# abacus-gene/paml

Hardware: AMD Instinct MI355X
Metric: site-patterns/sec per lnL eval (codeml M0, 61 states) (higher is better)
Workload: dtype f64; 1 GPU; codeml M0 61-state, 16 taxa x 1000000 synthetic codon patterns sharded over the GPUs (BASELINE configs[3]); classes=1, kernel=mfma64_jit, parallelism=pattern-shard x1, RCCL all-reduce inside the engine, patterns_rank0=1000000

## Files before the change

### include/paml_amd.h

```cpp
#ifndef PAML_AMD_H
#define PAML_AMD_H

#ifdef __cplusplus
extern "C" {
#endif

typedef struct paml_amd_engine paml_amd_engine;

enum {
   PAML_AMD_OK = 0,
   PAML_AMD_EINVAL = -1,
   PAML_AMD_ENOMEM = -2,
   PAML_AMD_EHIP = -3,
   PAML_AMD_EUNSUPPORTED = -4,
   PAML_AMD_ENOCONV = -5
};

enum {
   PAML_AMD_KEEP_PARTIALS = 1,
   PAML_AMD_JIT = 2,
   PAML_AMD_SHARD = 4
};

enum { PAML_AMD_EIGEN_UVROOT = 0, PAML_AMD_EIGEN_CIJK = 1, PAML_AMD_EIGEN_K80 = 2, PAML_AMD_EIGEN_JC69LIKE = 3, PAML_AMD_EIGEN_QMAT = 4 };
// ... 68 lines not shown
                        const double *qfactor, const double *freqK, const double *rate, double *lnL, double *lnf);

int paml_amd_eval_branch(paml_amd_engine *e, int node_b, int n_t, const double *t, const double *branch,
                         const double *gene_rate, double *lnL, double *dlnL, double *ddlnL);
int paml_amd_branch_counters(const paml_amd_engine *e, long *n_calls, long *n_nodes_recomputed);
long paml_amd_branch_coef_hits(const paml_amd_engine *e);
long paml_amd_branch_refill_kernels(const paml_amd_engine *e);
double paml_amd_branch_kernel_ms(paml_amd_engine *e);
int paml_amd_get_branch_partials(paml_amd_engine *e, double *out, long cap, long *rows, int *cols);

int paml_amd_node_posterior(paml_amd_engine *e, int node, const double *branch, const double *gene_rate, double *post);

int paml_amd_get_pmat(paml_amd_engine *e, int gene, int iclass, int node, double *P);
int paml_amd_get_partials(paml_amd_engine *e, int node, int iclass, double *conP);
int paml_amd_get_scale(paml_amd_engine *e, int node, int iclass, double *scale);
int paml_amd_get_partial_sums(paml_amd_engine *e, double *out, int cap);

int paml_amd_profile(paml_amd_engine *e, int enable);
int paml_amd_profile_read(paml_amd_engine *e, double *ms_pmat, double *ms_prune, double *ms_reduce, long *n_evals);

int paml_amd_counters(const paml_amd_engine *e, long *n_eval, long *n_pmat);

int paml_amd_cherry_tables(const paml_amd_engine *e, long *n_tabulated, long *bytes);
int paml_amd_subtree_tables(const paml_amd_engine *e, long *n_tabulated, int *nodes, long *u, int cap, long *bytes, long *blocks_left, long *n_computed);
int paml_amd_subtree_order(const paml_amd_engine *e, int *in_use, long *n_computed, double *host_seconds);
int paml_amd_gather_walk(const paml_amd_engine *e, int *in_use, long *n_tiles, long *n_rows, int *R, long *n_computed, double *host_seconds);

int paml_amd_debug_program(int n_tips, int n_nodes, int root, const int *sons_ptr, const int *sons,
                           const unsigned char *scale_node, int keep_partials, const unsigned char *clean,
                           int *ops_out, int cap, int *max_stack);

int paml_amd_debug_branch_plan(int n_tips, int n_nodes, int root, const int *sons_ptr, const int *sons, const unsigned char *scale_node,
                               int n_calls, const int *node_b, const double *branch, int *ends_out, int *up_out, unsigned char *clean_out,
                               int *ops_out, int cap);

int paml_amd_debug_code_order(int n_states, int n_codes, const int *n_chara, const unsigned char *chara_map, const unsigned char *z,
                              long nz, int *order_out);

int paml_amd_debug_jit(int n_tips, int n_nodes, int root, const int *sons_ptr, const int *sons,
                       const unsigned char *scale_node, char *text_out, int cap, int compile);

int paml_amd_debug_jit_tables(int n_tips, int n_nodes, int root, const int *sons_ptr, const int *sons, const unsigned char *scale_node,
                              int max_tabs, char *text_out, int cap, int *stream_out, int stream_cap, int *n_stream, int *tabs_out,
                              int tabs_cap);

int paml_amd_debug_subtree_classes(int n_tips, int n_nodes, int root, const int *sons_ptr, const int *sons, const unsigned char *z, long n_patt,
                                   int n_codes, unsigned int *u_out, unsigned int *cls_out);
// ... 141 lines not shown
```

### paml_amd/csrc/engine_core.hip

```cpp
#include "engine_state.h"
#include "eigen_kernels.h"

namespace paml_amd {
int launch_eigen_qrev(paml_amd_engine *e, EigenQrevArgs a, int n_sets)
{
   if (!e->eigen_attr_set) {
      for (const void *fn : {(const void *)eigen_qrev_kernel<0>, (const void *)eigen_qrev_kernel<20>, (const void *)eigen_qrev_kernel<60>, (const void *)eigen_qrev_kernel<62>})
         HIPCHK(hipFuncSetAttribute(fn, hipFuncAttributeMaxDynamicSharedMemorySize, (int)EIG_LDS_BYTES));
      e->eigen_attr_set = true;
   }
   static const int sweep_limit = getenv("PAML_AMD_EIGEN_SWEEP_LIMIT") ? std::max(1, atoi(getenv("PAML_AMD_EIGEN_SWEEP_LIMIT"))) : 40;
   a.max_sweeps = sweep_limit;
   const int N_even = (a.n + 1) & ~1;
   if (N_even == 62) hipLaunchKernelGGL(eigen_qrev_kernel<62>, dim3(n_sets), dim3(EIG_NT), EIG_LDS_BYTES, e->stream, a);
   else if (N_even == 60) hipLaunchKernelGGL(eigen_qrev_kernel<60>, dim3(n_sets), dim3(EIG_NT), EIG_LDS_BYTES, e->stream, a);
   else if (N_even == 20) hipLaunchKernelGGL(eigen_qrev_kernel<20>, dim3(n_sets), dim3(EIG_NT), EIG_LDS_BYTES, e->stream, a);
   else hipLaunchKernelGGL(eigen_qrev_kernel<0>, dim3(n_sets), dim3(EIG_NT), EIG_LDS_BYTES, e->stream, a);
   HIPCHK(hipGetLastError());
   return 0;
}
}

extern "C" {

// ... 680 lines not shown
   for (size_t i = 0; i + 5 < e->ev_used.size(); i += 6)
      for (int k = 0; k < 3; k++) {
         float ms = 0;
         if (hipEventElapsedTime(&ms, e->ev_used[i + 2 * k], e->ev_used[i + 2 * k + 1]) == hipSuccess) acc[k] += ms;
      }
   for (DevEvent &ev : e->ev_used) e->ev_pool.push_back(std::move(ev));
   e->ev_used.clear();
   if (ms_pmat) *ms_pmat = acc[0];
   if (ms_prune) *ms_prune = acc[1];
   if (ms_reduce) *ms_reduce = acc[2];
   if (n_evals) *n_evals = e->prof_evals;
   e->prof_evals = 0;
   return 0;
}

int paml_amd_cherry_tables(const paml_amd_engine *e, long *n_tabulated, long *bytes)
{
   if (!e) return PAML_AMD_EINVAL;
   if (n_tabulated) *n_tabulated = e->last_ctab_n;
   if (bytes) *bytes = e->last_ctab_bytes;
   return 0;
}

int paml_amd_subtree_tables(const paml_amd_engine *e, long *n_tabulated, int *nodes, long *u, int cap, long *bytes, long *blocks_left, long *n_computed)
{
   if (!e) return PAML_AMD_EINVAL;
   if (n_tabulated) *n_tabulated = e->last_stab_n;
   for (long i = 0; i < e->last_stab_n && i < cap && i < (long)e->sub.sel.size(); i++) {
      if (nodes) nodes[i] = e->sub.sel[i];
      if (u) u[i] = (long)e->sub.u[e->sub.sel[i]];
   }
   if (bytes) *bytes = e->last_stab_bytes;
   if (blocks_left) *blocks_left = e->last_stab_blocks;
   if (n_computed) *n_computed = e->sub.n_computed;
   return 0;
}

int paml_amd_subtree_order(const paml_amd_engine *e, int *in_use, long *n_computed, double *host_seconds)
{
   if (!e) return PAML_AMD_EINVAL;
   if (in_use) *in_use = (e->last_stab_n && e->sub.ordered) ? 1 : 0;
   if (n_computed) *n_computed = e->sub.n_order_computed;
   if (host_seconds) *host_seconds = e->sub.order_host_s;
   return 0;
}

int paml_amd_gather_walk(const paml_amd_engine *e, int *in_use, long *n_tiles, long *n_rows, int *R, long *n_computed, double *host_seconds)
{
   if (!e) return PAML_AMD_EINVAL;
// ... 19 lines not shown
```

### paml_amd/csrc/engine_eval.hip

```cpp
#include "engine_state.h"
#include "kernels_pmat.h"
#include "kernels_prune.h"
#include "kernels_reduce.h"

namespace paml_amd {

int build_tiles(paml_amd_engine *e)
{
   std::vector<int2> tiles;
   for (int g = 0; g < e->n_genes; g++)
      for (int h = e->gene_off[g]; h < e->gene_off[g + 1]; h += e->tile_patt) tiles.push_back(make_int2(g, h));
   e->n_tiles = (int)tiles.size();
   HIPCHK(upload(e->d_tiles, tiles.data(), tiles.size(), e->stream));
   const int tf = e->kk == KK_MFMA64 ? GATHER_WAVES * 16 : 256;
   std::vector<int2> tfull;
   for (int g = 0; g < e->n_genes; g++)
      for (int h = e->gene_off[g]; h < e->gene_off[g + 1]; h += tf) tfull.push_back(make_int2(g, h));
   e->n_tiles_full = (int)tfull.size();
   HIPCHK(upload(e->d_tiles_full, tfull.data(), tfull.size(), e->stream));
   if (e->kk == KK_MFMA64) {
      std::vector<int> g0(tiles.size());
      size_t k = 0;
      int base = 0;
      for (int g = 0; g < e->n_genes; g++) {
// ... 177 lines not shown
};

int begin_eval(paml_amd_engine *e, Eval &c)
{
   if (!(e->have_tips && e->have_tree && e->have_pi && e->have_classes))
      return fail(e, PAML_AMD_EINVAL, "eval before set_tips/set_tree/set_pi/set_classes");
   if (e->eigen.empty()) return fail(e, PAML_AMD_EINVAL, "eval before any set_eigen_*");
   c.keep = (e->flags & PAML_AMD_KEEP_PARTIALS) != 0;
   if (c.clean && (!c.keep || !e->partials_valid))
      return fail(e, PAML_AMD_EINVAL, "eval_dirty needs PAML_AMD_KEEP_PARTIALS and a previous full evaluation");
   c.B = c.bs ? c.bs->B : 1; c.Km = e->K; c.K = c.Km * c.B; c.G = e->n_genes; c.psets = c.G * c.K;
   if (c.B > 1 && (c.keep || c.clean)) return fail(e, PAML_AMD_EUNSUPPORTED, "eval_batch: not with PAML_AMD_KEEP_PARTIALS");
   c.new_prog = !e->prog_valid || c.clean;
   if (c.new_prog) {
      e->prog = build_program(e->tree, c.keep, c.clean);
      e->prog_valid = (c.clean == nullptr);
      if (int rc = check_stack_depth(e, e->prog)) { e->prog_valid = false; return rc; }
   }
   return 0;
}

int setup_streams(paml_amd_engine *e, Eval &c)
{
   c.want_pipe = c.want_pipe && (e->kk == KK_MFMA64 || (e->kk == KK_VALU20 && e->want_m20)) && (long)e->n_patt * e->K >= 100000;
   c.pipe = c.want_pipe && e->pipe_ok && !c.bs && !c.clean && !c.keep && !c.new_prog && !e->eigen_dirty;
   c.dual = c.pipe && e->dual_ok && !e->profiling;
   c.lane = c.dual ? e->red_slot : 0;
   if (c.dual && c.lane && !e->sb[c.lane - 1]) HIPCHK(create_engine_stream(&e->sb[c.lane - 1]));
   if (c.dual)
      if (int rc = ensure_side_stream(e)) return rc;
   c.ms = c.lane ? e->sb[c.lane - 1] : e->stream;
   if (c.want_pipe && !e->s2) {
      for (DevEvent &ev : e->ev_setread) HIPCHK(ev.ensure(hipEventDisableTiming));
      for (int i = 0; i < paml_amd_engine::NPSET - 1; i++) e->spare[i].id = i + 1;
      HIPCHK(create_engine_stream(&e->s2));
      HIPCHK(e->ev_entry[0].ensure(hipEventDisableTiming));
      HIPCHK(e->ev_entry[1].ensure(hipEventDisableTiming));
      HIPCHK(e->ev_pmat.ensure(hipEventDisableTiming));
   }
   c.ps = e->stream;
   if (c.pipe) {
      c.ps = e->s2;
      if (e->have_prev_entry && !(c.dual && e->dual_run)) HIPCHK(hipStreamWaitEvent(e->s2, e->ev_entry[e->entry_sel ^ 1], 0));
      const int nid = e->spare[e->spare_head].id;
      if (c.dual && e->setread_rec[nid]) HIPCHK(hipStreamWaitEvent(e->s2, e->ev_setread[nid], 0));
   }
   c.skip_entry = c.dual && e->dual_run;
   e->dual_run = c.dual;
   return 0;
}

int stage_inputs(paml_amd_engine *e, Eval &c, InlineVec &iv)
{
   const int B = c.B, Km = c.Km, G = c.G, nn = e->tree.n_nodes;
   const BatchSpec *const bs = c.bs;
   std::vector<EigenDev> tab;
// ... 377 lines not shown
         e->fused_threads = 256 * pl.CW;
      }
      if (!jit_ok) {
         int r = obtain_kernel(e, e->jit_slot, &e->jit, true, "v" + std::to_string(n) + ":" + jit_program_key(e->prog, e->n_tips),
                               [&]() { return jit_generate_valu(e->prog, n); }, JIT_WAIT_CALLER, "valu", &jit_ok);
         if (r) return r;
      }
   }
   if (e->want_m20 && !c.clean && jit_m20_supported(e->prog, e->n_tips, G)) {
      int r = obtain_kernel(e, e->jit_slot, &e->jit, true, std::string("m20c") + std::to_string(e->n_codes) + (G > 1 ? "g:" : ":") + jit_program_key(e->prog, e->n_tips),
                            [&]() { return jit_generate_m20(e->prog, e->n_tips, e->n_codes, G > 1 ? 2 : 1); }, JIT_WAIT_CALLER, "m20", &jit_ok);
      if (r) return r;
      second = jit_ok;
   }
   *out = PruneKernel(3 * e->kk + (second ? 2 : (jit_ok ? 1 : 0)));
   return 0;
}

int ensure_buffers(paml_amd_engine *e, Eval &c)
{
   if (c.pipe) {
      paml_amd_engine::PSet &sp = e->spare[e->spare_head];
      std::swap(e->d_rowmajor, sp.rowmajor); std::swap(e->d_pint, sp.pint); std::swap(e->d_ptip, sp.ptip); std::swap(e->d_pcol, sp.pcol);
      std::swap(e->d_ctab, sp.ctab);
      std::swap(e->d_stab, sp.stab);
      std::swap(e->pset, sp.id);
      e->spare_head = (e->spare_head + 1) % (paml_amd_engine::NPSET - 1);
   }
   if (int rc = ensure_pmat_buffers(e, c.psets, e->kk == KK_VALU20 && e->want_m20, e->kk == KK_MFMA64)) return rc;
   if (e->kernel != PK_MFMA64_JIT) e->n_ctab = e->n_stab = 0;
   e->last_stab_n = e->n_stab;
   e->last_stab_bytes = e->n_stab ? (long)((size_t)c.K * e->sub.rows * CHERRY_ROW_BYTES) : 0;
   e->last_stab_blocks = e->n_stab ? (long)(e->sub.sp.prog.stream.size() / 2) : -1;
   if (e->n_stab) HIPCHK(e->d_stab.ensure((size_t)e->last_stab_bytes / sizeof(double)));
   e->last_ctab_n = e->n_ctab;
   e->last_ctab_bytes = (long)((size_t)c.K * e->n_ctab * cherry_table_bytes(e->n_codes));
   if (e->n_ctab) HIPCHK(e->d_ctab.ensure((size_t)e->last_ctab_bytes / sizeof(double)));
   HIPCHK(e->d_fhK.ensure((size_t)c.K * e->n_patt));
   c.n_blocks = e->n_tiles * c.K;
   if (c.keep) {
      const int n_int = e->tree.n_nodes - e->n_tips;
      size_t words = e->kk == KK_MFMA64 ? (size_t)c.K * n_int * e->part_groups() * 1024 + (size_t)std::max(e->mfma_waves, 8) * 1024
                                        : (size_t)c.K * n_int * e->n_patt * e->n;
      HIPCHK(e->d_partials.ensure(words));
      HIPCHK(e->d_scalef.ensure((size_t)c.K * std::max(1, e->tree.n_scale) * e->n_patt));
   }
   return stack_overflow(e, e->prog, c.n_blocks, e->mfma_waves, &c.overflow);
}

int run_pmat(paml_amd_engine *e, Eval &c, const InlineVec &iv)
{
   const int B = c.B, Km = c.Km, G = c.G, nn = e->tree.n_nodes;
   const BatchSpec *const bs = c.bs;
   PmatArgs pa = pmat_args(e, e->tree.root, e->d_label.p, e->kk == KK_MFMA64 ? 1 : (e->kernel == PK_MFMA4X20_JIT ? 2 : 0),
                           e->kk == KK_MFMA64 ? e->d_pcol.p : nullptr);
   if (c.pipe) { pa.branch = e->d2_branch.p; pa.gene_rate = e->d2_gene_rate.p; }
   pa.B = B; pa.branch_bs = nn; pa.gene_rate_bs = G;
   if (bs && bs->eigen_of) { pa.eigen_of = e->d_b_eigen_of.p; pa.eigen_of_bs = (long)G * Km * e->n_labels; }
   if (bs && bs->qfactor) { pa.qfactor = e->d_b_qfactor.p; pa.qfactor_bs = (long)Km * e->n_labels; }
   pa.npb = 1;
// ... 4 lines not shown
   e->pmat_B = B;
   if (pmat_mfma && !bs && c.use_inline && !e->rate_per_gene && !e->eigen.empty()) {
      if (!e->pres_valid) {
         std::vector<PmatRes> res((size_t)c.psets * nn);
         for (int g = 0; g < G; g++)
            for (int ir = 0; ir < Km; ir++)
               for (int v = 0; v < nn; v++) {
                  const int lab = e->tree.label.empty() ? 0 : e->tree.label[v];
                  const EigenHost &h = e->eigen[e->h_eigen_of[((size_t)g * Km + ir) * e->n_labels + lab]];
                  res[((size_t)g * Km + ir) * nn + v] = PmatRes{h.U.p, h.V.p, h.Root.p, e->class_rate[ir], e->h_qfactor[(size_t)ir * e->n_labels + lab],
                                                                e->tree.is_leaf(v) ? 1 : 0, 0};
               }
         HIPCHK(e->d_pres.ensure(res.size()));
         HIPCHK(hipMemcpyAsync(e->d_pres.p, res.data(), res.size() * sizeof(PmatRes), hipMemcpyHostToDevice, c.ps));
         e->pres_valid = true;
      }
      pa.res = e->d_pres.p;
   }
   mark_on(e, c.ps);
   bool small_pmat = e->kk != KK_MFMA64 && e->n <= 5;
   for (const EigenHost &h : e->eigen) small_pmat = small_pmat && h.kind != PAML_AMD_EIGEN_QMAT;
   launch_pmat(pa, iv, nn, c.psets, small_pmat, c.ps, pmat_mfma);
   if (e->n_ctab) {
      CherryTabArgs ca{};
      ca.n_codes = e->n_codes; ca.n_nodes = nn; ca.n_tabs = e->n_ctab; ca.tip_words = (long)tip_words(e);
      ca.pint = e->d_pint.p; ca.ptip = e->d_ptip.p; ca.pcol = e->d_pcol.p; ca.ctab = e->d_ctab.p;
      for (int i = 0; i < e->n_ctab; i++) { ca.tabs[3 * i] = e->cherry.tabs[i].tip_a; ca.tabs[3 * i + 1] = e->cherry.tabs[i].tip_b; ca.tabs[3 * i + 2] = e->cherry.tabs[i].node; }
      const size_t lds = (size_t)(3 * 4096 + 64) * sizeof(double);
      if (!e->ctab_attr_set) {
         HIPCHK(hipFuncSetAttribute((const void *)cherry_table_kernel<true>, hipFuncAttributeMaxDynamicSharedMemorySize, (int)lds));
         HIPCHK(hipFuncSetAttribute((const void *)cherry_table_kernel<false>, hipFuncAttributeMaxDynamicSharedMemorySize, (int)lds));
         HIPCHK(hipFuncSetAttribute((const void *)cherry_table_kernel<false, 15>, hipFuncAttributeMaxDynamicSharedMemorySize, (int)lds));
         e->ctab_attr_set = true;
      }
      const dim3 g((e->n_codes * e->n_codes + 127) / 128, e->n_ctab, c.K);
      if (e->n == 61) hipLaunchKernelGGL(cherry_table_kernel<true>, g, dim3(512), lds, c.ps, ca);
      else if (e->n == 60) hipLaunchKernelGGL((cherry_table_kernel<false, 15>), g, dim3(512), lds, c.ps, ca);
      else hipLaunchKernelGGL(cherry_table_kernel<false>, g, dim3(512), lds, c.ps, ca);
   }
   if (e->n_stab) {
      const paml_amd_engine::Subtree &sb = e->sub;
      SubtreeTabArgs sa{};
      sa.n_codes = e->n_codes; sa.n_nodes = nn; sa.n_ctab = e->n_ctab; sa.tip_words = (long)tip_words(e); sa.stab_rows = sb.rows;
      sa.pint = e->d_pint.p; sa.ptip = e->d_ptip.p; sa.pcol = e->d_pcol.p; sa.ctab = e->d_ctab.p;
      sa.nodes = sb.d_nodes.p; sa.sidx = sb.d_sidx.p; sa.stab = e->d_stab.p;
      const size_t lds_full = (size_t)(3 * 4096 + 64) * sizeof(double), lds_small = (size_t)(4096 + 64) * sizeof(double);
      if (!e->stab_attr_set) {
         HIPCHK(hipFuncSetAttribute((const void *)subtree_table_kernel<true>, hipFuncAttributeMaxDynamicSharedMemorySize, (int)lds_full));
         HIPCHK(hipFuncSetAttribute((const void *)subtree_table_kernel<false>, hipFuncAttributeMaxDynamicSharedMemorySize, (int)lds_full));
         HIPCHK(hipFuncSetAttribute((const void *)subtree_table_kernel<false, 15>, hipFuncAttributeMaxDynamicSharedMemorySize, (int)lds_full));
         e->stab_attr_set = true;
      }
      for (int l = 0; l < sb.sp.levels; l++) {
         sa.first = sb.level_first[l];
         sa.small = sb.level_small[l] ? 1 : 0;
         const size_t lds = sa.small ? lds_small : lds_full;
         const dim3 g(sb.level_tiles[l], sb.level_first[l + 1] - sb.level_first[l], c.K);
         if (e->n == 61) hipLaunchKernelGGL(subtree_table_kernel<true>, g, dim3(512), lds, c.ps, sa);
         else if (e->n == 60) hipLaunchKernelGGL((subtree_table_kernel<false, 15>), g, dim3(512), lds, c.ps, sa);
         else hipLaunchKernelGGL(subtree_table_kernel<false>, g, dim3(512), lds, c.ps, sa);
      }
   }
   mark_on(e, c.ps);
   if (c.pipe) {
      HIPCHK(hipEventRecord(e->ev_pmat, e->s2));
      HIPCHK(hipStreamWaitEvent(c.ms, e->ev_pmat, 0));
   }
   if (c.want_pipe && !c.skip_entry) {
// ... 47 lines not shown
   c.slot_waited = false;
   if (c.offload) {
      if (int rc = ensure_side_stream(e)) return rc;
      if (int rc = wait_slot(e, c)) return rc;
   }
   if ((size_t)B * RED_TICKET_WORDS > e->d_red_counter.cap) {
      HIPCHK(e->d_red_counter.ensure((size_t)std::max(B, 64) * RED_TICKET_WORDS));
      HIPCHK(hipMemsetAsync(e->d_red_counter.p, 0, e->d_red_counter.cap * sizeof(int), c.ms));
   }
   HIPCHK(e->d_out.ensure(B));
   if (c.want_lnf) HIPCHK(e->d_lnf.ensure((size_t)B * e->n_patt));
   return 0;
}

int run_prune(paml_amd_engine *e, Eval &c)
{
   const PruneKernel k = e->kernel;
   const int B = c.B, K = c.K, G = c.G, n_blocks = c.n_blocks;
   const BatchSpec *const bs = c.bs;
   if (pk_module(k) && e->tree.n_scale) HIPCHK(e->d_fscale.ensure((size_t)K * e->n_patt));
   PruneArgs pr = prune_args(e, e->prog, K, e->d_ops.p, false, e->tree.n_scale, c.keep, e->d_partials.p, e->d_scalef.p, c.overflow);
   if (k == PK_MFMA4X20_JIT) { pr.pint = e->d_pint.p; pr.pcol = e->d_rowmajor.p; }
   pr.fhK = e->fhk_slot(e->last_fhk).p;
   if (k == PK_MFMA64_JIT && e->n_ctab) { pr.ctab = e->d_ctab.p; pr.n_ctab = e->n_ctab; }
   if (k == PK_MFMA64_JIT && e->n_stab) {
      pr.stab = e->d_stab.p; pr.stab_rows = e->sub.rows; pr.stab_meta = e->sub.d_meta.p;
      pr.ztiles = e->sub.d_ztiles.p; pr.zt_bytes = e->sub.zt_bytes;
      pr.order = e->sub.ordered ? e->sub.d_order.p : nullptr;
   }
   const paml_amd_engine::Subtree &gsb = e->sub;
   const bool gather = k == PK_MFMA64_JIT && e->n_stab && !bs && gather_walk_wanted() && e->env.prof_ops.empty() && !e->env.prof_tiles && gsb.gw_ok &&
                       gsb.gw_sel_gen == gsb.sel_gen && gsb.gw_ordered == gsb.ordered && gsb.gw_tiles > 0 && gsb.d_gw_desc.p;
   e->last_gw = gather;
   if (gather) {
      pr.gw_desc = gsb.d_gw_desc.p; pr.gw_tiles = (int)gsb.gw_tiles; pr.gw_desc_bytes = gather_desc_bytes(gsb.gw_R); pr.gw_R = gsb.gw_R;
      for (int i = 0; i < 4; i++) { pr.gw_kind[i] = gsb.gw_kind[i]; pr.gw_id[i] = gsb.gw_id[i]; }
   }
   const int nb = (e->n_patt + e->chunk - 1) / e->chunk;
   if (pk_forms_reduction(k)) {
      pr.Km = c.Km; pr.chunk = e->chunk; pr.first_chunk = e->first_chunk; pr.nb_stride = e->nb_global;
      pr.want_fhk = (c.want_fhk || e->tree.n_scale) ? 1 : 0;
      pr.freqK = (bs && bs->freqK) ? e->d_b_freqK.p : e->d_freqK.p; pr.freqK_bs = (bs && bs->freqK) ? c.Km : 0;
      pr.lnf = c.want_lnf ? e->d_lnf.p : nullptr;
      pr.red_partial = e->part_slot(c.slot).p; pr.red_out = c.d_lnL_out ? c.d_lnL_out : e->d_out.p; pr.nb_local = nb;
      if (int rc = wait_slot(e, c)) return rc;
      pr.red_counter = k == PK_MFMA64_COOPJIT ? e->d_red_counter.p : nullptr;
   }
   if (!e->env.prof_ops.empty()) {
      const int prof_stride = std::max((int)e->prog.ops.size() + 3, e->env.prof_tiles ? 96 : 0);
// ... 51 lines not shown
      break;
   }
   case PK_MFMA4X20_JIT: {
      int grid = std::min(std::max(K, cus / K * K), e->n_tiles * K);
      if (two_streams && G == 1) {
         const int units = std::min(e->n_tiles * 8, (e->n_patt + 31) / 32), g78 = e->n_cu * 7 / 8 / K * K;
         auto rounds = [&](int g) { return ((units + g / K - 1) / (g / K) + 7) / 8; };
         if (g78 >= K && g78 < grid && rounds(g78) == rounds(grid)) grid = g78;
      }
      HIPCHK(hipModuleLaunchKernel(e->jit.fn, std::max(grid / K, G > 1 ? G : 1) * K, 1, 1, 512, 1, 1, 0, ms, params, nullptr));
      break;
   }
   case PK_VALU4_JIT: case PK_VALU5_JIT: case PK_VALU20_JIT:
      HIPCHK(hipModuleLaunchKernel(e->jit.fn, n_blocks, 1, 1, 256, 1, 1, 0, ms, params, nullptr));
      break;
   case PK_MFMA64_GATHER: case PK_VALU4: case PK_VALU5: case PK_VALU20:
      launch_prune_full(e, e->prog.max_stack, n_blocks, pr, ms);
      break;
   }
   mark(e);
   if (c.want_pipe && e->env.dual) {
      HIPCHK(hipEventRecord(e->ev_setread[e->pset], ms));
      e->setread_rec[e->pset] = true;
   }
   return 0;
}

int dump_op_stamps(paml_amd_engine *e, const Eval &c)
{
   if (e->env.prof_ops.empty() || e->env.prof_tiles) return 0;
   std::vector<unsigned long long> hp((size_t)3 * e->prof_blocks * e->prof_stride);
   HIPCHK(hipMemcpyAsync(hp.data(), e->d_prof, hp.size() * 8, hipMemcpyDeviceToHost, c.ms));
   HIPCHK(hipStreamSynchronize(c.ms));
   if (FILE *f = fopen(e->env.prof_ops.c_str(), "wb")) {
      int hdr[2] = {e->prof_blocks, e->prof_stride};
      fwrite(hdr, sizeof(int), 2, f);
      std::vector<int> codes;
      for (auto &o : e->prog.ops) codes.push_back(o.code);
      codes.resize(e->prof_stride - 3, 0);
      fwrite(codes.data(), sizeof(int), codes.size(), f);
      fwrite(hp.data(), 8, hp.size(), f);
      fclose(f);
   }
   return 0;
}

// ... 233 lines not shown
```

### paml_amd/csrc/engine_state.h

```cpp
#pragma once
#include <hip/hip_runtime.h>

#include <algorithm>
#include <cmath>
#include <cstdio>
#include <cstdlib>
#include <cstring>
#include <string>
#include <atomic>
#include <functional>
#include <memory>
#include <mutex>
#include <set>
#include <thread>
#include <vector>

#include <dlfcn.h>
#include <unistd.h>
#include <rccl/rccl.h>

#include "../../include/paml_amd.h"
#include "jit.h"
#include "jit_cache.h"
#include "kernel_args.h"
// ... 103 lines not shown
inline Rccl &rccl()
{
   static Rccl r;
   return r;
}

inline int red_chunk(long n_global) { return (int)std::max<long>(256, ((n_global + 1023) / 1024 + 255) / 256 * 256); }

struct EnvCfg {
   bool offload = false;
   bool dual = true;
   bool no_coef_cache = false;
   bool no_branch_eig = false;
   bool no_coop = false;
   bool jit_sync = false, jit_strict = false, no_m20 = false;
   int comm_cus = -1, lanes = 0;
   int cherry_tables = -1;
   long cherry_min_patt = 32768, cherry_cap_mb = 192;
   int subtree_tables = -1;
   double subtree_max_frac = 0.5;
   long subtree_cap_mb = 2048;
   int subtree_order = 1;
   int gather_R = 128;
   int subtree_rows = 1;
   std::string jit_dump, prof_ops;
   int prof_tid = 0;
   bool prof_tiles = false;
   bool comm_stats = false;
   void read()
   {
      if (const char *v = getenv("PAML_AMD_COOP")) no_coop = atoi(v) == 0;
      offload = getenv("PAML_AMD_OFFLOAD") != nullptr;
      if (const char *v = getenv("PAML_AMD_DUAL")) dual = atoi(v) != 0;
      jit_sync = getenv("PAML_AMD_JIT_SYNC") != nullptr;
      jit_strict = getenv("PAML_AMD_JIT_STRICT") != nullptr;
      no_m20 = getenv("PAML_AMD_NO_M20") != nullptr;
      no_branch_eig = getenv("PAML_AMD_NO_BRANCH_EIG") != nullptr;
      no_coef_cache = getenv("PAML_AMD_NO_COEF_CACHE") != nullptr;
      if (const char *v = getenv("PAML_AMD_COMM_CUS")) comm_cus = atoi(v);
      comm_stats = getenv("PAML_AMD_COMM_STATS") != nullptr;
      if (const char *v = getenv("PAML_AMD_LANES")) lanes = atoi(v);
      if (const char *v = getenv("PAML_AMD_CHERRY_TABLES")) cherry_tables = atoi(v) != 0 ? 1 : 0;
      if (const char *v = getenv("PAML_AMD_CHERRY_MIN_PATT")) cherry_min_patt = atol(v);
      if (const char *v = getenv("PAML_AMD_CHERRY_CAP_MB")) cherry_cap_mb = std::max(0L, atol(v));
      if (const char *v = getenv("PAML_AMD_SUBTREE_TABLES")) subtree_tables = atoi(v) != 0 ? 1 : 0;
      if (const char *v = getenv("PAML_AMD_SUBTREE_MAX_FRAC")) subtree_max_frac = std::max(0.0, atof(v));
      if (const char *v = getenv("PAML_AMD_SUBTREE_CAP_MB")) subtree_cap_mb = std::max(0L, atol(v));
      if (const char *v = getenv("PAML_AMD_SUBTREE_ORDER")) subtree_order = std::max(0, std::min(2, atoi(v)));
      if (const char *v = getenv("PAML_AMD_SUBTREE_ROWS")) subtree_rows = atoi(v) != 0 ? 1 : 0;
      if (const char *v = getenv("PAML_AMD_GATHER_R")) gather_R = std::max(8, std::min(128, atoi(v))) & ~1;
      if (const char *v = getenv("PAML_AMD_JIT_DUMP")) jit_dump = v;
      if (const char *v = getenv("PAML_AMD_PROF_OPS")) prof_ops = v;
      if (const char *v = getenv("PAML_AMD_PROF_TID")) prof_tid = atoi(v);
      prof_tiles = getenv("PAML_AMD_PROF_TILES") != nullptr;
   }
};

}

using namespace paml_amd;

inline void worker_threads_list(std::thread *th, bool add)
{
   static std::mutex m;
   static std::vector<std::pair<std::thread *, pid_t>> live;
   static const bool registered = (atexit([]() { worker_threads_list(nullptr, false); }), true);
   (void)registered;
   std::vector<std::thread *> to_join;
   {
      std::lock_guard<std::mutex> lk(m);
      if (th && add) live.emplace_back(th, getpid());
      else if (th) live.erase(std::remove_if(live.begin(), live.end(), [th](const std::pair<std::thread *, pid_t> &e) { return e.first == th; }), live.end());
      else
// ... 88 lines not shown
   int tiles_built_for = 0;
   void swap_tile_stash()
   {
      TileStash &t = tile_stash;
      std::swap(t.built_for, tiles_built_for); std::swap(t.n_tiles, n_tiles); std::swap(t.zt_bytes, zt_bytes); std::swap(t.zt_key, zt_key);
      std::swap(t.tiles, d_tiles); std::swap(t.group0, d_tile_group0); std::swap(t.ztip_of, d_ztip_of); std::swap(t.ztiles, d_ztiles);
   }
   int part_groups() const { return n_tiles_full * GATHER_WAVES; }
   DevBuf<double> d_pi_plain;
   DevBuf<double> d_weights, d_pi, d_freqK, d_rate, d_qfactor, d_branch, d_gene_rate;
   std::vector<int> gene_off;
   int n_tiles = 0, n_pi = 1;

   TreeDesc tree;
   Program prog;
   bool prog_valid = false;
   DevBuf<Op> d_ops;
   DevBuf<int> d_stream;
   Staging stage;
   JitKernel jit;
   CherryProgram cherry;
   std::string cherry_key;
   int cherry_n = 0;
   DevBuf<double> d_ctab;
   int n_ctab = 0;
   bool ctab_attr_set = false;
   long last_ctab_n = 0, last_ctab_bytes = 0;
   struct Subtree {
      struct Key {
         long tips_gen = -1, tree_gen = -1, cherry_gen = -1, cap_mb = -1;
         double frac = -1;
         int K = -1;
         bool operator==(const Key &o) const { return tips_gen == o.tips_gen && tree_gen == o.tree_gen && cherry_gen == o.cherry_gen && cap_mb == o.cap_mb && frac == o.frac && K == o.K; }
      } made_for;
      long sel_gen = 0, zt_sel_gen = -1;
      int zt_tiles = 0, zt_tile_patt = 0;
      std::vector<unsigned int> u;
      std::vector<char> done;
      std::vector<std::vector<unsigned int>> cls, son_cls;
      std::vector<int> sel;
      SubtreeProgram sp;
      std::vector<int> level_first;
      std::vector<int> level_tiles;
      long rows = 0;
      long n_computed = 0;
      long n_order_computed = 0;
      bool ordered = false;
      std::vector<std::vector<unsigned int>> rowmap;
      std::vector<char> level_small;
      DevBuf<int> d_order;
      long order_sel_gen = -1;
      double order_host_s = 0;
      int zt_bytes = 0;
      DevBuf<SubtreeNodeDev> d_nodes;
      DevBuf<unsigned int> d_sidx, d_top_cls;
      DevBuf<int> d_meta;
      DevBuf<unsigned char> d_ztiles;
      std::vector<unsigned int> h_order;
      DevBuf<unsigned char> d_gw_desc;
      long gw_sel_gen = -1, gw_plan_gen = -1, gw_tiles = 0, gw_rows = 0, gw_computed = 0;
      int gw_R = 0, gw_nlk = 0, gw_kind[4] = {0, 0, 0, 0}, gw_id[4] = {0, 0, 0, 0};
      bool gw_ok = false, gw_ordered = false;
      double gw_host_s = 0;
   } sub;
   bool gw_attr_set = false, last_gw = false;
   std::vector<unsigned char> h_z, h_wflag;
   long tips_gen = 0, tree_gen = 0, cherry_gen = 0;
   DevBuf<double> d_stab;
   int n_stab = 0;
   bool stab_attr_set = false;
   long last_stab_n = 0, last_stab_bytes = 0, last_stab_blocks = -1;
   std::vector<JitKernel> jit_pool;
   std::vector<std::pair<std::string, int>> jit_seen;
   void jit_retire()
   {
      if (jit.mod && jit.fn) {
         if (jit_pool.size() >= 8) { (void)hipModuleUnload(jit_pool.front().mod); jit_pool.erase(jit_pool.begin()); }
         jit_pool.push_back(jit);
      }
      else if (jit.mod) (void)hipModuleUnload(jit.mod);
      jit = JitKernel();
   }
   bool jit_recall(const std::string &key)
   {
      if (jit.fn && jit.key == key) return true;
      for (size_t i = 0; i < jit_pool.size(); i++)
         if (jit_pool[i].key == key && jit_pool[i].fn) {
            const JitKernel k = jit_pool[i];
            jit_pool.erase(jit_pool.begin() + i);
            jit_retire();
            jit = k;
            return true;
         }
      return false;
   }
   int jit_count_request(const std::string &key)
   {
      for (auto &kv : jit_seen)
         if (kv.first == key) return ++kv.second;
      if (jit_seen.size() >= 64) jit_seen.erase(jit_seen.begin());
      jit_seen.emplace_back(key, 1);
      return 1;
   }
   bool jit_enabled = false;
   bool small20 = false;
   JitKernel jit_coop;
   bool coopj_enabled = true;
   bool pipe_ok = false;
   hipStream_t s2 = nullptr;
   DevEvent ev_entry[2], ev_pmat;
   int entry_sel = 0;
   bool have_prev_entry = false;
   static constexpr int NPSET = 6;
   struct PSet { DevBuf<double> rowmajor, pint, ptip, pcol, ctab, stab; int id = 0; } spare[NPSET - 1];
   int spare_head = 0;
   DevBuf<double> d2_branch, d2_gene_rate;
   hipStream_t sb[MAXL - 1] = {};
   DevEvent ev_setread[NPSET];
   bool setread_rec[NPSET] = {};
   int pset = 0;
   bool dual_ok = false, dual_run = false;
   bool jit_forced = false;
   struct JitJob {
      std::thread th;
      std::atomic<int> state{0};
      std::string key, src, log;
      std::vector<char> code;
      JitJob() { worker_threads_list(&th, true); }
      ~JitJob() { if (th.joinable()) th.join(); worker_threads_list(&th, false); }
   };
   struct JitSlot {
      std::unique_ptr<JitJob> job;
      std::set<std::string> failed;
   };
   JitSlot jit_slot, coop_slot, bjit_slot;

   std::vector<EigenHost> eigen;
// ... 269 lines not shown
```

### paml_amd/csrc/kernels_reduce.h

```cpp
#pragma once
#include <hip/hip_runtime.h>

#include "kernel_args.h"

namespace paml_amd {

__device__ __forceinline__ double pattern_lnf(const ReduceArgs &a, int h)
{
   if (a.mode == PAML_AMD_MODE_LFUN) return a.fhK[h];
   double fh;
   if (a.n_scale) {
      int it = 0;
      for (int ir = 1; ir < a.K; ir++)
         if (a.fhK[(long)ir * a.n_patt + h] > a.fhK[(long)it * a.n_patt + h]) it = ir;
      const double t = a.fhK[(long)it * a.n_patt + h];
      fh = 0;
      for (int ir = 0; ir < a.K; ir++) fh += a.freqK[ir] * exp(a.fhK[(long)ir * a.n_patt + h] - t);
      return t + log(fh);
   }
   fh = 0;
   for (int ir = 0; ir < a.K; ir++) fh += a.freqK[ir] * a.fhK[(long)ir * a.n_patt + h];
   if (fh <= 0) fh = 1e-300;
   return log(fh);
}

__global__ __launch_bounds__(256) void reduce_stage1(ReduceArgs a)
{
   if (blockIdx.y) {
      const long off = (long)blockIdx.y * a.K * a.n_patt;
      a.fhK += off;
      if (a.fscale) a.fscale += off;
      a.freqK += blockIdx.y * a.freqK_bs;
      a.partial += (long)blockIdx.y * a.nb_stride;
      if (a.lnf) a.lnf += (long)blockIdx.y * a.n_patt;
   }
   const int lo = blockIdx.x * a.chunk;
   const int hi = min(a.n_patt, lo + a.chunk);
   double acc = 0;
   for (int h = lo + threadIdx.x; h < hi; h += 256) {
      double v = 0;
      if (a.weights[h] > 0) {
         if (a.raw && (a.mode == PAML_AMD_MODE_LFUN || a.n_scale)) {
            for (int ir = 0; ir < a.K; ir++) {
               const long ix = (long)ir * a.n_patt + h;
               a.fhK[ix] = log(a.fhK[ix]) + (a.n_scale ? a.fscale[ix] : 0.0);
            }
         }
         v = pattern_lnf(a, h);
         acc += v * a.weights[h];
      }
      if (a.lnf) a.lnf[h] = v;
   }
   red_block_finish(acc, a.partial, a.first_chunk + blockIdx.x, a.nb_stride, a.out + blockIdx.y, nullptr);
}

__global__ __launch_bounds__(256) void reduce_stage2(const double *partial, int nb, double *out)
{
   __shared__ double sw[4];
   double acc = 0;
   partial += (long)blockIdx.x * nb;
   out += blockIdx.x;
   for (int i = threadIdx.x; i < nb; i += 256) acc += partial[i];
#pragma unroll
   for (int off = 32; off >= 1; off >>= 1) acc += __shfl_xor(acc, off);
   if ((threadIdx.x & 63) == 0) sw[threadIdx.x >> 6] = acc;
   __syncthreads();
   if (threadIdx.x == 0) *out = (sw[0] + sw[1]) + (sw[2] + sw[3]);
}

}
```

### paml_amd/engine.py

```python
from __future__ import annotations

import ctypes as C
import os
import subprocess

import numpy as np

from .problem import EIGEN_CIJK, EIGEN_JC69LIKE, EIGEN_K80, EIGEN_QMAT, EIGEN_UVROOT, Problem

_HERE = os.path.dirname(os.path.abspath(__file__))
LIB_PATH = os.environ.get("PAML_AMD_LIB") or os.path.join(_HERE, "lib", "libpaml_amd.so")
CSRC = os.path.join(_HERE, "csrc")
KEEP_PARTIALS = 1
JIT = 2
SHARD = 4

EXPORTS = [
    "paml_amd_set_gene_class_rates", "paml_amd_get_branch_partials", "paml_amd_create", "paml_amd_destroy", "paml_amd_last_error", "paml_amd_set_stream", "paml_amd_set_tips",
    "paml_amd_set_tree", "paml_amd_set_pi", "paml_amd_set_eigen_uvroot", "paml_amd_set_eigen_cijk",
    "paml_amd_set_eigen_qrev_batch", "paml_amd_set_eigen_qrev_batch_sparse", "paml_amd_set_eigen_warm_start", "paml_amd_get_eigen", "paml_amd_eigen_counters", "paml_amd_set_eigen_k80", "paml_amd_set_eigen_jc69like", "paml_amd_set_eigen_qmat", "paml_amd_set_classes", "paml_amd_eval",
    "paml_amd_eval_batch", "paml_amd_eval_adg", "paml_amd_beb_grid", "paml_amd_beb_grid_classes", "paml_amd_compress_patterns", "paml_amd_eval_device", "paml_amd_eval_dirty", "paml_amd_eval_branch", "paml_amd_node_posterior", "paml_amd_get_pmat", "paml_amd_get_partials", "paml_amd_get_scale",
    "paml_amd_device_count", "paml_amd_set_device", "paml_amd_shard_bounds", "paml_amd_max_ranks", "paml_amd_flush", "paml_amd_eigen_status", "paml_amd_comm_unique_id", "paml_amd_comm_init", "paml_amd_comm_destroy", "paml_amd_comm_info", "paml_amd_comm_library", "paml_amd_comm_stats", "paml_amd_get_partial_sums", "paml_amd_branch_counters", "paml_amd_branch_coef_hits", "paml_amd_branch_refill_kernels", "paml_amd_branch_kernel_ms",
    "paml_amd_jit_prebuild", "paml_amd_profile", "paml_amd_profile_read", "paml_amd_counters", "paml_amd_kernel_name", "paml_amd_debug_program", "paml_amd_debug_jit",
    "paml_amd_cherry_tables", "paml_amd_debug_jit_tables",
# ... 1 lines not shown
    "paml_amd_gather_walk", "paml_amd_debug_gather_tiles",
    "paml_amd_debug_code_order", "paml_amd_debug_branch_plan", "paml_amd_debug_device_bytes",
    "paml_amd_pairset_create", "paml_amd_pairset_destroy", "paml_amd_pairset_get_counts", "paml_amd_pairset_set_pi", "paml_amd_pairset_set_pattern",
    "paml_amd_pairset_eval", "paml_amd_pairset_failed", "paml_amd_pairset_counters",
    "paml_amd_rell_replicates", "paml_amd_rell_info",
    "paml_amd_simulate", "paml_amd_simulate_info",
    "paml_amd_ancestral_marginal", "paml_amd_ancestral_joint", "paml_amd_ancestral_info",
    "paml_amd_gradient", "paml_amd_gradient_info",
    "paml_amd_curvature", "paml_amd_curvature_info",
    "paml_amd_hessian", "paml_amd_hessian_info",
    "paml_amd_model_gradient", "paml_amd_model_gradient_info", "paml_amd_model_gradient_segment", "paml_amd_model_gradient_sizes",
    "paml_amd_subst_counts", "paml_amd_subst_counts_info",
    "paml_amd_nni_scores", "paml_amd_nni_info", "paml_amd_nni_list",
    "paml_amd_edge_scores", "paml_amd_edge_info", "paml_amd_edge_list",
    "paml_amd_relabel_scores", "paml_amd_relabel_info",
    "paml_amd_placement_scores", "paml_amd_placement_info",
    "paml_amd_attach_scores", "paml_amd_attach_info",
    "paml_amd_spr_scores", "paml_amd_spr_info", "paml_amd_spr_list",
]


class EngineError(RuntimeError):
    pass


UNIT_FLAGS = {}
EXTRA_FLAGS = os.environ.get("PAML_AMD_EXTRA_FLAGS", "").split()
UNITS = ("engine_core", "engine_comm", "engine_eval", "engine_branch", "engine_beb", "engine_jitdbg", "engine_compress", "engine_pairwise", "engine_rell", "engine_simulate", "engine_ancestral", "engine_gradient", "engine_curvature", "engine_hessian", "engine_modelgrad", "engine_counts", "engine_nni", "engine_place", "engine_attach", "engine_spr", "engine_edge", "engine_relabel")


def build(force: bool = False, verbose: bool = False) -> str:
    import glob
    from concurrent.futures import ThreadPoolExecutor
    hdrs = glob.glob(os.path.join(CSRC, "*.h")) + [os.path.join(os.path.dirname(_HERE), "include", "paml_amd.h")]
    newest_hdr = max(os.path.getmtime(h) for h in hdrs)
    hipcc = os.environ.get("HIPCC", "/opt/rocm/bin/hipcc")
    objdir = os.path.join(os.path.dirname(LIB_PATH), "obj")
    os.makedirs(objdir, exist_ok=True)
    jobs = []
    for u in UNITS:
        src, obj = os.path.join(CSRC, u + ".hip"), os.path.join(objdir, u + ".o")
        if force or not os.path.exists(obj) or os.path.getmtime(obj) < max(newest_hdr, os.path.getmtime(src)):
            jobs.append([hipcc, "--offload-arch=gfx950", "-O3", "-std=c++17", "-fPIC"] + UNIT_FLAGS.get(u, []) + EXTRA_FLAGS + ["-c", src, "-o", obj])
    objs = [os.path.join(objdir, u + ".o") for u in UNITS]
    if not jobs and os.path.exists(LIB_PATH) and all(os.path.getmtime(o) <= os.path.getmtime(LIB_PATH) for o in objs):
        return LIB_PATH
# ... 573 lines not shown
        return a

    def get_scale(self, node, iclass=0):
        a = np.zeros(self.n_patt)
        self._chk(self._L.paml_amd_get_scale(self._h, node, iclass, _p(a)))
        return a

    def profile(self, on=True):
        self._chk(self._L.paml_amd_profile(self._h, int(on)))

    def profile_read(self):
        a, b, c, n = C.c_double(), C.c_double(), C.c_double(), C.c_long()
        self._chk(self._L.paml_amd_profile_read(self._h, C.byref(a), C.byref(b), C.byref(c), C.byref(n)))
        return dict(ms_pmat=a.value, ms_prune=b.value, ms_reduce=c.value, n_evals=n.value)

    def cherry_tables(self):
        a, b = C.c_long(), C.c_long()
        self._L.paml_amd_cherry_tables.argtypes = [C.c_void_p, C.POINTER(C.c_long), C.POINTER(C.c_long)]
        self._chk(self._L.paml_amd_cherry_tables(self._h, C.byref(a), C.byref(b)))
        return a.value, b.value

    def subtree_tables(self):
        cap = 256
        n, by, bl, nc = C.c_long(), C.c_long(), C.c_long(), C.c_long()
        nodes, u = np.zeros(cap, dtype=np.int32), np.zeros(cap, dtype=np.int64)
        self._L.paml_amd_subtree_tables.argtypes = [C.c_void_p, C.POINTER(C.c_long), C.c_void_p, C.c_void_p, C.c_int] + [C.POINTER(C.c_long)] * 3
        self._chk(self._L.paml_amd_subtree_tables(self._h, C.byref(n), _p(nodes), _p(u), cap, C.byref(by), C.byref(bl), C.byref(nc)))
        k = min(n.value, cap)
        return dict(nodes=nodes[:k].tolist(), u=u[:k].tolist(), bytes=by.value, blocks_left=bl.value, n_computed=nc.value)

    def subtree_order(self):
        use, nc, sec = C.c_int(), C.c_long(), C.c_double()
        self._L.paml_amd_subtree_order.argtypes = [C.c_void_p, C.POINTER(C.c_int), C.POINTER(C.c_long), C.POINTER(C.c_double)]
        self._chk(self._L.paml_amd_subtree_order(self._h, C.byref(use), C.byref(nc), C.byref(sec)))
        return dict(in_use=bool(use.value), n_computed=nc.value, host_seconds=sec.value)

    def gather_walk(self):
        use, nt, nr, r, nc, sec = C.c_int(), C.c_long(), C.c_long(), C.c_int(), C.c_long(), C.c_double()
        self._L.paml_amd_gather_walk.argtypes = [C.c_void_p, C.POINTER(C.c_int), C.POINTER(C.c_long), C.POINTER(C.c_long), C.POINTER(C.c_int), C.POINTER(C.c_long),
                                                 C.POINTER(C.c_double)]
        self._chk(self._L.paml_amd_gather_walk(self._h, C.byref(use), C.byref(nt), C.byref(nr), C.byref(r), C.byref(nc), C.byref(sec)))
        return dict(in_use=bool(use.value), tiles=nt.value, rows=nr.value, R=r.value, n_computed=nc.value, host_seconds=sec.value)

    def counters(self):
        a, b = C.c_long(), C.c_long()
        self._L.paml_amd_counters(self._h, C.byref(a), C.byref(b))
        return dict(n_eval=a.value, n_pmat=b.value)


class PairSet:

    def __init__(self, eng: Engine, pairs):
# ... 513 lines not shown
```

Baseline: 5.339 billion site-patterns/s.

## Decouple cherry/subtree table buffers into event-guarded rotating sets; unroll reduce stage

Moves the cherry and subtree table buffers out of the pipelined P-matrix spare sets into their own ring of 2 to 6 table sets, sized by table bytes. Each set carries a read event so the next table build waits only on the prune that last used that set, not on the whole previous eval. This is meant to let table construction overlap more with the previous prune. Separately, reduce_stage1 gains a register-unrolled path for K<=4 that loads four patterns per thread before computing logs, to raise memory-level parallelism. The pipeline threshold also becomes an env knob. The extra table sets use more device memory.

```diff
diff --git a/include/paml_amd.h b/include/paml_amd.h
--- a/include/paml_amd.h
+++ b/include/paml_amd.h
@@ -114,7 +114,8 @@
 int paml_amd_counters(const paml_amd_engine *e, long *n_eval, long *n_pmat);
 
 int paml_amd_cherry_tables(const paml_amd_engine *e, long *n_tabulated, long *bytes);
-int paml_amd_subtree_tables(const paml_amd_engine *e, long *n_tabulated, int *nodes, long *u, int cap, long *bytes, long *blocks_left, long *n_computed);
+int paml_amd_subtree_tables(const paml_amd_engine *e, long *n_tabulated, int *nodes, long *u, int cap, long *bytes, long *blocks_left, long *n_computed,
+                            long *table_sets);
 int paml_amd_subtree_order(const paml_amd_engine *e, int *in_use, long *n_computed, double *host_seconds);
 int paml_amd_gather_walk(const paml_amd_engine *e, int *in_use, long *n_tiles, long *n_rows, int *R, long *n_computed, double *host_seconds);
 
diff --git a/paml_amd/csrc/engine_core.hip b/paml_amd/csrc/engine_core.hip
--- a/paml_amd/csrc/engine_core.hip
+++ b/paml_amd/csrc/engine_core.hip
@@ -726,9 +726,11 @@
    return 0;
 }
 
-int paml_amd_subtree_tables(const paml_amd_engine *e, long *n_tabulated, int *nodes, long *u, int cap, long *bytes, long *blocks_left, long *n_computed)
-{
-   if (!e) return PAML_AMD_EINVAL;
+int paml_amd_subtree_tables(const paml_amd_engine *e, long *n_tabulated, int *nodes, long *u, int cap, long *bytes, long *blocks_left, long *n_computed,
+                            long *table_sets)
+{
+   if (!e) return PAML_AMD_EINVAL;
+   if (table_sets) *table_sets = e->last_ctab_n ? e->n_tabsets : 0;
    if (n_tabulated) *n_tabulated = e->last_stab_n;
    for (long i = 0; i < e->last_stab_n && i < cap && i < (long)e->sub.sel.size(); i++) {
       if (nodes) nodes[i] = e->sub.sel[i];
diff --git a/paml_amd/csrc/engine_eval.hip b/paml_amd/csrc/engine_eval.hip
--- a/paml_amd/csrc/engine_eval.hip
+++ b/paml_amd/csrc/engine_eval.hip
@@ -223,7 +223,7 @@
 
 int setup_streams(paml_amd_engine *e, Eval &c)
 {
-   c.want_pipe = c.want_pipe && (e->kk == KK_MFMA64 || (e->kk == KK_VALU20 && e->want_m20)) && (long)e->n_patt * e->K >= 100000;
+   c.want_pipe = c.want_pipe && (e->kk == KK_MFMA64 || (e->kk == KK_VALU20 && e->want_m20)) && (long)e->n_patt * e->K >= e->env.pipe_min;
    c.pipe = c.want_pipe && e->pipe_ok && !c.bs && !c.clean && !c.keep && !c.new_prog && !e->eigen_dirty;
    c.dual = c.pipe && e->dual_ok && !e->profiling;
    c.lane = c.dual ? e->red_slot : 0;
@@ -233,6 +233,7 @@
    c.ms = c.lane ? e->sb[c.lane - 1] : e->stream;
    if (c.want_pipe && !e->s2) {
       for (DevEvent &ev : e->ev_setread) HIPCHK(ev.ensure(hipEventDisableTiming));
+      for (paml_amd_engine::TabSet &ts : e->tabset) HIPCHK(ts.ev_read.ensure(hipEventDisableTiming));
       for (int i = 0; i < paml_amd_engine::NPSET - 1; i++) e->spare[i].id = i + 1;
       HIPCHK(create_engine_stream(&e->s2));
       HIPCHK(e->ev_entry[0].ensure(hipEventDisableTiming));
@@ -656,8 +657,6 @@
    if (c.pipe) {
       paml_amd_engine::PSet &sp = e->spare[e->spare_head];
       std::swap(e->d_rowmajor, sp.rowmajor); std::swap(e->d_pint, sp.pint); std::swap(e->d_ptip, sp.ptip); std::swap(e->d_pcol, sp.pcol);
-      std::swap(e->d_ctab, sp.ctab);
-      std::swap(e->d_stab, sp.stab);
       std::swap(e->pset, sp.id);
       e->spare_head = (e->spare_head + 1) % (paml_amd_engine::NPSET - 1);
    }
@@ -666,10 +665,17 @@
    e->last_stab_n = e->n_stab;
    e->last_stab_bytes = e->n_stab ? (long)((size_t)c.K * e->sub.rows * CHERRY_ROW_BYTES) : 0;
    e->last_stab_blocks = e->n_stab ? (long)(e->sub.sp.prog.stream.size() / 2) : -1;
-   if (e->n_stab) HIPCHK(e->d_stab.ensure((size_t)e->last_stab_bytes / sizeof(double)));
    e->last_ctab_n = e->n_ctab;
    e->last_ctab_bytes = (long)((size_t)c.K * e->n_ctab * cherry_table_bytes(e->n_codes));
-   if (e->n_ctab) HIPCHK(e->d_ctab.ensure((size_t)e->last_ctab_bytes / sizeof(double)));
+   if (e->n_ctab) {
+      e->n_tabsets = e->table_sets_for(e->last_ctab_bytes + e->last_stab_bytes);
+      e->tab_cur = (e->tab_cur + (c.pipe ? 1 : 0)) % e->n_tabsets;
+      paml_amd_engine::TabSet &ts = e->tabs();
+      const size_t cw = (size_t)e->last_ctab_bytes / sizeof(double), sw = (size_t)e->last_stab_bytes / sizeof(double);
+      if ((cw > ts.ctab.cap || sw > ts.stab.cap) && ts.read_rec) HIPCHK(hipEventSynchronize(ts.ev_read));
+      HIPCHK(ts.ctab.ensure(cw));
+      if (e->n_stab) HIPCHK(ts.stab.ensure(sw));
+   }
    HIPCHK(e->d_fhK.ensure((size_t)c.K * e->n_patt));
    c.n_blocks = e->n_tiles * c.K;
    if (c.keep) {
@@ -720,9 +726,11 @@
    for (const EigenHost &h : e->eigen) small_pmat = small_pmat && h.kind != PAML_AMD_EIGEN_QMAT;
    launch_pmat(pa, iv, nn, c.psets, small_pmat, c.ps, pmat_mfma);
    if (e->n_ctab) {
+      paml_amd_engine::TabSet &ts = e->tabs();
+      if (ts.read_rec) HIPCHK(hipStreamWaitEvent(c.ps, ts.ev_read, 0));
       CherryTabArgs ca{};
       ca.n_codes = e->n_codes; ca.n_nodes = nn; ca.n_tabs = e->n_ctab; ca.tip_words = (long)tip_words(e);
-      ca.pint = e->d_pint.p; ca.ptip = e->d_ptip.p; ca.pcol = e->d_pcol.p; ca.ctab = e->d_ctab.p;
+      ca.pint = e->d_pint.p; ca.ptip = e->d_ptip.p; ca.pcol = e->d_pcol.p; ca.ctab = ts.ctab.p;
       for (int i = 0; i < e->n_ctab; i++) { ca.tabs[3 * i] = e->cherry.tabs[i].tip_a; ca.tabs[3 * i + 1] = e->cherry.tabs[i].tip_b; ca.tabs[3 * i + 2] = e->cherry.tabs[i].node; }
       const size_t lds = (size_t)(3 * 4096 + 64) * sizeof(double);
       if (!e->ctab_attr_set) {
@@ -740,8 +748,8 @@
       const paml_amd_engine::Subtree &sb = e->sub;
       SubtreeTabArgs sa{};
       sa.n_codes = e->n_codes; sa.n_nodes = nn; sa.n_ctab = e->n_ctab; sa.tip_words = (long)tip_words(e); sa.stab_rows = sb.rows;
-      sa.pint = e->d_pint.p; sa.ptip = e->d_ptip.p; sa.pcol = e->d_pcol.p; sa.ctab = e->d_ctab.p;
-      sa.nodes = sb.d_nodes.p; sa.sidx = sb.d_sidx.p; sa.stab = e->d_stab.p;
+      sa.pint = e->d_pint.p; sa.ptip = e->d_ptip.p; sa.pcol = e->d_pcol.p; sa.ctab = e->tabs().ctab.p;
+      sa.nodes = sb.d_nodes.p; sa.sidx = sb.d_sidx.p; sa.stab = e->tabs().stab.p;
       const size_t lds_full = (size_t)(3 * 4096 + 64) * sizeof(double), lds_small = (size_t)(4096 + 64) * sizeof(double);
       if (!e->stab_attr_set) {
          HIPCHK(hipFuncSetAttribute((const void *)subtree_table_kernel<true>, hipFuncAttributeMaxDynamicSharedMemorySize, (int)lds_full));
@@ -835,9 +843,9 @@
    PruneArgs pr = prune_args(e, e->prog, K, e->d_ops.p, false, e->tree.n_scale, c.keep, e->d_partials.p, e->d_scalef.p, c.overflow);
    if (k == PK_MFMA4X20_JIT) { pr.pint = e->d_pint.p; pr.pcol = e->d_rowmajor.p; }
    pr.fhK = e->fhk_slot(e->last_fhk).p;
-   if (k == PK_MFMA64_JIT && e->n_ctab) { pr.ctab = e->d_ctab.p; pr.n_ctab = e->n_ctab; }
+   if (k == PK_MFMA64_JIT && e->n_ctab) { pr.ctab = e->tabs().ctab.p; pr.n_ctab = e->n_ctab; }
    if (k == PK_MFMA64_JIT && e->n_stab) {
-      pr.stab = e->d_stab.p; pr.stab_rows = e->sub.rows; pr.stab_meta = e->sub.d_meta.p;
+      pr.stab = e->tabs().stab.p; pr.stab_rows = e->sub.rows; pr.stab_meta = e->sub.d_meta.p;
       pr.ztiles = e->sub.d_ztiles.p; pr.zt_bytes = e->sub.zt_bytes;
       pr.order = e->sub.ordered ? e->sub.d_order.p : nullptr;
    }
@@ -935,6 +943,10 @@
    if (c.want_pipe && e->env.dual) {
       HIPCHK(hipEventRecord(e->ev_setread[e->pset], ms));
       e->setread_rec[e->pset] = true;
+   }
+   if (c.want_pipe && k == PK_MFMA64_JIT && e->n_ctab) {
+      HIPCHK(hipEventRecord(e->tabs().ev_read, ms));
+      e->tabs().read_rec = true;
    }
    return 0;
 }
diff --git a/paml_amd/csrc/engine_state.h b/paml_amd/csrc/engine_state.h
--- a/paml_amd/csrc/engine_state.h
+++ b/paml_amd/csrc/engine_state.h
@@ -149,6 +149,8 @@
    long subtree_cap_mb = 2048;
    int subtree_order = 1;
    int gather_R = 128;
+   int table_sets = 0;
+   long pipe_min = 100000;
    int subtree_rows = 1;
    std::string jit_dump, prof_ops;
    int prof_tid = 0;
@@ -176,6 +178,8 @@
       if (const char *v = getenv("PAML_AMD_SUBTREE_ORDER")) subtree_order = std::max(0, std::min(2, atoi(v)));
       if (const char *v = getenv("PAML_AMD_SUBTREE_ROWS")) subtree_rows = atoi(v) != 0 ? 1 : 0;
       if (const char *v = getenv("PAML_AMD_GATHER_R")) gather_R = std::max(8, std::min(128, atoi(v))) & ~1;
+      if (const char *v = getenv("PAML_AMD_TABLE_SETS")) table_sets = std::max(1, std::min(6, atoi(v)));
+      if (const char *v = getenv("PAML_AMD_PIPE_MIN")) pipe_min = std::max(0L, atol(v));
       if (const char *v = getenv("PAML_AMD_JIT_DUMP")) jit_dump = v;
       if (const char *v = getenv("PAML_AMD_PROF_OPS")) prof_ops = v;
       if (const char *v = getenv("PAML_AMD_PROF_TID")) prof_tid = atoi(v);
@@ -310,7 +314,6 @@
    CherryProgram cherry;
    std::string cherry_key;
    int cherry_n = 0;
-   DevBuf<double> d_ctab;
    int n_ctab = 0;
    bool ctab_attr_set = false;
    long last_ctab_n = 0, last_ctab_bytes = 0;
@@ -354,7 +357,10 @@
    bool gw_attr_set = false, last_gw = false;
    std::vector<unsigned char> h_z, h_wflag;
    long tips_gen = 0, tree_gen = 0, cherry_gen = 0;
-   DevBuf<double> d_stab;
+   struct TabSet { DevBuf<double> ctab, stab; DevEvent ev_read; bool read_rec = false; } tabset[6];
+   int n_tabsets = 1, tab_cur = 0;
+   TabSet &tabs() { return tabset[tab_cur]; }
+   int table_sets_for(long bytes) const { return env.table_sets ? env.table_sets : (bytes <= (256L << 20) ? 2 : 6); }
    int n_stab = 0;
    bool stab_attr_set = false;
    long last_stab_n = 0, last_stab_bytes = 0, last_stab_blocks = -1;
@@ -400,7 +406,7 @@
    int entry_sel = 0;
    bool have_prev_entry = false;
    static constexpr int NPSET = 6;
-   struct PSet { DevBuf<double> rowmajor, pint, ptip, pcol, ctab, stab; int id = 0; } spare[NPSET - 1];
+   struct PSet { DevBuf<double> rowmajor, pint, ptip, pcol; int id = 0; } spare[NPSET - 1];
    int spare_head = 0;
    DevBuf<double> d2_branch, d2_gene_rate;
    hipStream_t sb[MAXL - 1] = {};
diff --git a/paml_amd/csrc/kernels_reduce.h b/paml_amd/csrc/kernels_reduce.h
--- a/paml_amd/csrc/kernels_reduce.h
+++ b/paml_amd/csrc/kernels_reduce.h
@@ -24,6 +24,69 @@
    return log(fh);
 }
 
+template <int KR>
+__device__ __forceinline__ double pattern_lnf_regs(const ReduceArgs &a, const double (&x)[KR])
+{
+   if (a.mode == PAML_AMD_MODE_LFUN) return x[0];
+   double fh = 0;
+   if (a.n_scale) {
+      double t = x[0];
+#pragma unroll
+      for (int ir = 1; ir < KR; ir++)
+         if (ir < a.K && x[ir] > t) t = x[ir];
+#pragma unroll
+      for (int ir = 0; ir < KR; ir++)
+         if (ir < a.K) fh = fma(a.freqK[ir], exp(x[ir] - t), fh);
+      return t + log(fh);
+   }
+#pragma unroll
+   for (int ir = 0; ir < KR; ir++)
+      if (ir < a.K) fh = fma(a.freqK[ir], x[ir], fh);
+   if (fh <= 0) fh = 1e-300;
+   return log(fh);
+}
+
+template <int KR>
+__device__ __forceinline__ void reduce_group(const ReduceArgs &a, int h0, int hi, bool rawlog, double &acc)
+{
+   constexpr int U = 4;
+   double w[U], x[U][KR], s[U][KR];
+#pragma unroll
+   for (int j = 0; j < U; j++) {
+      const int h = h0 + 256 * j;
+      w[j] = h < hi ? a.weights[h] : 0.0;
+   }
+#pragma unroll
+   for (int j = 0; j < U; j++) {
+      const int h = h0 + 256 * j;
+#pragma unroll
+      for (int ir = 0; ir < KR; ir++) {
+         const bool there = h < hi && ir < a.K;
+         x[j][ir] = there ? a.fhK[(long)ir * a.n_patt + h] : 1.0;
+         s[j][ir] = there && rawlog && a.n_scale ? a.fscale[(long)ir * a.n_patt + h] : 0.0;
+      }
+   }
+#pragma unroll
+   for (int j = 0; j < U; j++) {
+      const int h = h0 + 256 * j;
+      if (h >= hi) break;
+      double v = 0;
+      if (w[j] > 0) {
+         if (rawlog) {
+#pragma unroll
+            for (int ir = 0; ir < KR; ir++)
+               if (ir < a.K) {
+                  x[j][ir] = log(x[j][ir]) + (a.n_scale ? s[j][ir] : 0.0);
+                  a.fhK[(long)ir * a.n_patt + h] = x[j][ir];
+               }
+         }
+         v = pattern_lnf_regs<KR>(a, x[j]);
+         acc = fma(v, w[j], acc);
+      }
+      if (a.lnf) a.lnf[h] = v;
+   }
+}
+
 __global__ __launch_bounds__(256) void reduce_stage1(ReduceArgs a)
 {
    if (blockIdx.y) {
@@ -36,21 +99,27 @@
    }
    const int lo = blockIdx.x * a.chunk;
    const int hi = min(a.n_patt, lo + a.chunk);
+   const bool rawlog = a.raw && (a.mode == PAML_AMD_MODE_LFUN || a.n_scale);
    double acc = 0;
-   for (int h = lo + threadIdx.x; h < hi; h += 256) {
-      double v = 0;
-      if (a.weights[h] > 0) {
-         if (a.raw && (a.mode == PAML_AMD_MODE_LFUN || a.n_scale)) {
-            for (int ir = 0; ir < a.K; ir++) {
-               const long ix = (long)ir * a.n_patt + h;
-               a.fhK[ix] = log(a.fhK[ix]) + (a.n_scale ? a.fscale[ix] : 0.0);
+   if (a.K == 1)
+      for (int h0 = lo + threadIdx.x; h0 < hi; h0 += 4 * 256) reduce_group<1>(a, h0, hi, rawlog, acc);
+   else if (a.K <= 4)
+      for (int h0 = lo + threadIdx.x; h0 < hi; h0 += 4 * 256) reduce_group<4>(a, h0, hi, rawlog, acc);
+   else
+      for (int h = lo + threadIdx.x; h < hi; h += 256) {
+         double v = 0;
+         if (a.weights[h] > 0) {
+            if (rawlog) {
+               for (int ir = 0; ir < a.K; ir++) {
+                  const long ix = (long)ir * a.n_patt + h;
+                  a.fhK[ix] = log(a.fhK[ix]) + (a.n_scale ? a.fscale[ix] : 0.0);
+               }
             }
+            v = pattern_lnf(a, h);
+            acc += v * a.weights[h];
          }
-         v = pattern_lnf(a, h);
-         acc += v * a.weights[h];
+         if (a.lnf) a.lnf[h] = v;
       }
-      if (a.lnf) a.lnf[h] = v;
-   }
    red_block_finish(acc, a.partial, a.first_chunk + blockIdx.x, a.nb_stride, a.out + blockIdx.y, nullptr);
 }
 
diff --git a/paml_amd/engine.py b/paml_amd/engine.py
--- a/paml_amd/engine.py
+++ b/paml_amd/engine.py
@@ -47,6 +47,10 @@
 
 class EngineError(RuntimeError):
     pass
+
+
+class TableReport(dict):
+    table_sets = 0
 
 
 UNIT_FLAGS = {}
@@ -666,12 +670,14 @@
 
     def subtree_tables(self):
         cap = 256
-        n, by, bl, nc = C.c_long(), C.c_long(), C.c_long(), C.c_long()
+        n, by, bl, nc, ts = C.c_long(), C.c_long(), C.c_long(), C.c_long(), C.c_long()
         nodes, u = np.zeros(cap, dtype=np.int32), np.zeros(cap, dtype=np.int64)
-        self._L.paml_amd_subtree_tables.argtypes = [C.c_void_p, C.POINTER(C.c_long), C.c_void_p, C.c_void_p, C.c_int] + [C.POINTER(C.c_long)] * 3
-        self._chk(self._L.paml_amd_subtree_tables(self._h, C.byref(n), _p(nodes), _p(u), cap, C.byref(by), C.byref(bl), C.byref(nc)))
+        self._L.paml_amd_subtree_tables.argtypes = [C.c_void_p, C.POINTER(C.c_long), C.c_void_p, C.c_void_p, C.c_int] + [C.POINTER(C.c_long)] * 4
+        self._chk(self._L.paml_amd_subtree_tables(self._h, C.byref(n), _p(nodes), _p(u), cap, C.byref(by), C.byref(bl), C.byref(nc), C.byref(ts)))
         k = min(n.value, cap)
-        return dict(nodes=nodes[:k].tolist(), u=u[:k].tolist(), bytes=by.value, blocks_left=bl.value, n_computed=nc.value)
+        rep = TableReport(nodes=nodes[:k].tolist(), u=u[:k].tolist(), bytes=by.value, blocks_left=bl.value, n_computed=nc.value)
+        rep.table_sets = ts.value
+        return rep
 
     def subtree_order(self):
         use, nc, sec = C.c_int(), C.c_long(), C.c_double()
```

New measurement: 5.282 billion site-patterns/s. -1.1%, worse.
